# AlanLiangC/SPSNet

Hardware: NVIDIA B200
Metric: IA-SSD SA-backbone scenes/s (16k pts) (higher is better)
Workload: dtype fp16 operands / fp32 accumulate (split-fp16 hi+lo for K <= 64 chains and all Conv1d GEMMs); fp32 + int32 sampling

## Files before the change

spsnet_b200/csrc/sa_mma.cu:

```cuda
#include "sa_mma_common.cuh"
#include <stdlib.h>

namespace spsk {

template <int G, bool PROF, bool NP>
__global__ void __launch_bounds__(128 * G + 64 - (NP ? 32 : 0), G == 1 ? (NP ? 4 : 3) : 1)
sa_mma_kernel(const __grid_constant__ SaArgs a) {
    constexpr int W_PROD = NP ? -1 : 4 * G, W_MMA = NP ? 4 * G : 4 * G + 1;
    extern __shared__ __align__(128) uint8_t smem[];
    uint64_t *bars = reinterpret_cast<uint64_t *>(smem);
    uint32_t *tmem_slot = reinterpret_cast<uint32_t *>(smem + MM_HDR - 16);
    uint8_t *xa = smem + MM_HDR;
    uint8_t *xb = xa + a.xa_bytes;
    uint8_t *wst = xb + a.xb_bytes;
    const uint32_t bar0 = smem_u32(bars);
    auto W_FULL = [&](int s) { return bar0 + 8u * s; };
    auto W_EMPTY = [&](int s) { return bar0 + 8u * (MM_MAX_STAGES + s); };
    auto ACC_FULL = [&](int i) { return bar0 + 8u * (2 * MM_MAX_STAGES + i); };
    auto ACC_EMPTY = [&](int i) { return bar0 + 8u * (2 * MM_MAX_STAGES + 4 + i); };
    auto XR = [&](int buf, int c) { return bar0 + 8u * (2 * MM_MAX_STAGES + 8 + buf * MM_MAX_XC + c); };
    auto WL_FULL = [&](int s) { return bar0 + 8u * (2 * MM_MAX_STAGES + 8 + 2 * MM_MAX_XC + s); };
    auto WL_EMPTY = [&](int s) { return bar0 + 8u * (3 * MM_MAX_STAGES + 8 + 2 * MM_MAX_XC + s); };
    const uint32_t HID_DONE = bar0 + 8u * (4 * MM_MAX_STAGES + 8 + 2 * MM_MAX_XC);

// ... 39 lines not shown
                    { const long long t0 = pf.now(); mbar_wait(bar0 + ((R.z >> 10) & 1023u), ((R.z >> 20) ^ ((R.z >> 21) & tpar) ^ 1u) & 1u); pf.add(PF_PROD_W_EMPTY, t0); }
                    if (leader) {
                        const uint32_t full = bar0 + (R.z & 1023u), bytes = R.y & 0xFFFFu;
                        if (bytes == 0u || (PROF && (a.abl & 1) && tcount > 0u)) {
                            mbar_arrive(full);
                        } else {
                            mbar_expect_tx(full, bytes);
                            bulk_g2s(bar0 + ((R.y >> 16) << 4), a.wtiles + R.x, bytes, full);
                        }
                    }
                    __syncwarp();
                }
            }
            pf.flush(a.prof);
        } else {
            ProfT<PROF> pf;
            pf.init(a.prof != nullptr && leader);
            uint32_t tcount = 0;
            int ws = 0, ls = 0;
            uint32_t wph = 0u, lph = 0u;
            uint8_t *lst = ((nL - 2) & 1) ? xb : xa;
            for (int tile = blockIdx.x; tile < a.ntiles; tile += gridDim.x, ++tcount) {
                for (int l = 0; l < nL; ++l) {
                    const SaLayer &Ly = a.L[l];
                    const bool lring = a.lstages > 0 && l == nL - 1;
                    if (lring) { const long long t0 = pf.now(); mbar_wait(HID_DONE, tcount & 1u); pf.add(PF_PROD_HID, t0); }
                    for (int cci = 0; cci < Ly.n_cc; ++cci) {
                        const int cc = chunk_of(l, cci, Ly.n_cc);
                        const int ncols = min(128, Ly.cpad - cc * 128);
                        for (int kc = 0; kc < Ly.n_kc; ++kc) {
                            const int kw = min(64, Ly.wk - kc * 64);
                            const uint32_t bytes = (uint32_t)(ncols * kw * 2);
                            const uint8_t *src = a.wtiles + wtile_off(Ly, cc, kc, ncols);
                            uint32_t full, empty, dst, ph;
                            if (!lring) {
                                ph = wph;
                                full = W_FULL(ws); empty = W_EMPTY(ws); dst = smem_u32(wst + (size_t)ws * MM_STAGE_BYTES);
                                if (++ws == a.nstages) { ws = 0; wph ^= 1u; }
                            } else {
                                ph = lph;
                                full = WL_FULL(ls); empty = WL_EMPTY(ls); dst = smem_u32(lst + (size_t)ls * MM_STAGE_BYTES);
                                if (++ls == a.lstages) { ls = 0; lph ^= 1u; }
                            }
                            { const long long t0 = pf.now(); mbar_wait(empty, ph ^ 1u); pf.add(PF_PROD_W_EMPTY, t0); }
                            if (leader) {
                                mbar_expect_tx(full, bytes);
                                bulk_g2s(dst, src, bytes, full);
                            }
                            __syncwarp();
                        }
                    }
                }
            }
            pf.flush(a.prof);
        }
    } else if (warp == W_MMA) {
        if (a.narrow) {
            const bool leader = elect_one();
            if (NP && leader) {
                mbar_expect_tx(W_FULL(0), (uint32_t)a.w_total);
                for (int off = 0; off < a.w_total; off += MM_STAGE_BYTES) {
                    const int bytes = min(MM_STAGE_BYTES, a.w_total - off);
                    bulk_g2s(smem_u32(wst + off), a.wtiles + off, (uint32_t)bytes, W_FULL(0));
                }
            }
            uint32_t x_lo[MM_MAX_LAYERS], x_hi[MM_MAX_LAYERS], w_lo[MM_MAX_LAYERS], idesc[MM_MAX_LAYERS], tstride[MM_MAX_LAYERS];
            int nv[MM_MAX_LAYERS], nk1[MM_MAX_LAYERS], nk2[MM_MAX_LAYERS], nxc[MM_MAX_LAYERS], wkl[MM_MAX_LAYERS];
#pragma unroll
            for (int l = 0; l < MM_MAX_LAYERS; ++l) {
                const SaLayer &Ly = a.L[l < nL ? l : 0];
                const bool last = (l == nL - 1);
                x_lo[l] = umma_desc_lo(smem_u32((l & 1) ? xb : xa), 128u);
                x_hi[l] = umma_desc_hi((uint32_t)Ly.xw * 16u);
                w_lo[l] = umma_desc_lo(smem_u32(wst + Ly.w_off), 128u);
                tstride[l] = (uint32_t)(Ly.cpad * 64 * 2) >> 4;
                idesc[l] = last ? umma_idesc(128, MM_ROWS) : umma_idesc(128, Ly.cpad);
                nv[l] = Ly.vk >> 4;
                nk1[l] = a.split ? (Ly.kpad >> 4) : 0x7FFFFFFF;
                nk2[l] = a.split ? 2 * (Ly.kpad >> 4) : 0x7FFFFFFF;
                nxc[l] = Ly.n_xc;
                wkl[l] = Ly.wk;
            }
            mbar_wait(W_FULL(0), 0u);
            uint32_t job = 0;
            uint32_t xph[2] = {0u, 0u};
            const uint32_t nbmask = (uint32_t)a.nbuf - 1u;
            for (int tile = blockIdx.x; tile < a.ntiles; tile += gridDim.x) {
#pragma unroll
                for (int l = 0; l < MM_MAX_LAYERS; ++l) {
                    if (l < nL && l >= a.l0_fused) {
                        const bool last = (l == nL - 1);
                        const int buf = (int)(job & nbmask);
                        const uint32_t use = job >> a.nbuf_log2;
                        if (use > 0) mbar_wait(ACC_EMPTY(buf), (use - 1) & 1u);
                        for (int c = 0; c < nxc[l]; ++c) {
                            mbar_wait(XR(l & 1, c), (xph[l & 1] >> c) & 1u);
                            xph[l & 1] ^= (1u << c);
                        }
                        tc_fence_after();
                        if (leader) {
                            const uint32_t d_tmem = tmem_base + (uint32_t)(buf * 128);
                            for (int v = 0; v < nv[l]; ++v) {
                                const int xblk = v >= nk2[l] ? v - nk2[l] : v;
                                const int wblk = v >= nk1[l] ? v - nk1[l] : v;
                                const int kc = wblk >> 2, jj = wblk & 3;
                                const uint32_t kw = (uint32_t)min(64, wkl[l] - kc * 64);
                                const uint32_t wl = w_lo[l] + (uint32_t)kc * tstride[l] + 16u * (uint32_t)jj;
                                const uint32_t wh = umma_desc_hi(kw * 16u);
                                const uint32_t xl = x_lo[l] + 16u * (uint32_t)xblk;
                                if (!last) umma_f16_lohi(d_tmem, xl, x_hi[l], wl, wh, idesc[l], v ? 1u : 0u);
                                else umma_f16_lohi(d_tmem, wl, wh, xl, x_hi[l], idesc[l], v ? 1u : 0u);
                            }
                            umma_commit(ACC_FULL(buf));
                        }
                        __syncwarp();
                        ++job;
                    }
                }
            }
        } else if (a.sched_n > 0) {
            const bool leader = elect_one();
            ProfT<PROF> pf;
            pf.init(a.prof != nullptr && leader);
            const long long t_start = pf.now();
            uint32_t job = 0, tpar = 0u;
            const uint32_t nbmask = (uint32_t)a.nbuf - 1u;
            const int nent = a.sched_n;
            const uint32_t smem_base16 = bar0 >> 4;
            uint4 E = a.sched[0], R = a.ring[0];
            for (int tile = blockIdx.x; tile < a.ntiles; tile += gridDim.x, tpar ^= 1u) {
                int buf = 0;
                uint32_t d_tmem = tmem_base;
                for (int e = 0; e < nent; ++e) {
                    const int en = e + 1 < nent ? e + 1 : 0;
                    const uint4 En = a.sched[en], Rn = a.ring[en];
                    const uint32_t f = E.w;
                    if (f & SCH_FIRST_KC) {
                        buf = (int)(job & nbmask);
                        const uint32_t use = job >> a.nbuf_log2;
                        if (use > 0) { const long long t0 = pf.now(); mbar_wait(ACC_EMPTY(buf), (use - 1) & 1u); pf.add(PF_MMA_ACC_EMPTY, t0); }
                        d_tmem = tmem_base + (uint32_t)(buf * 128);
                    }
                    { const long long t0 = pf.now(); mbar_wait(bar0 + (R.z & 1023u), ((R.z >> 20) ^ ((R.z >> 21) & tpar)) & 1u); pf.add(PF_MMA_W_FULL, t0); }
                    if (R.z & (1u << 22)) {
                        const long long t0 = pf.now();
                        mbar_wait(bar0 + (R.w & 1023u), ((R.z >> 23) ^ ((R.z >> 24) & tpar)) & 1u);
                        if (R.z & (1u << 25)) mbar_wait(bar0 + (R.w >> 10), ((R.z >> 26) ^ ((R.z >> 27) & tpar)) & 1u);
                        pf.add(PF_MMA_XR, t0);
                    }
                    tc_fence_after();
                    if (leader) {
                        const long long t_i = pf.now();
                        const int nk16 = (PROF && (a.abl & 8) && (f & 15u)) ? 1 : (int)(f & 15u);
                        if (nk16) {
                            const uint32_t x_lo = E.x + smem_base16;
                            const uint32_t w_lo = (((smem_base16 + (R.y >> 16)) & 0x3FFFu) | ((128u >> 4) << 16));
                            const uint32_t w_lo2 = w_lo + ((f >> 16) & 2047u) - 64u;
                            const uint32_t x_hi = E.z & 0xFFFFu, w_hi = E.z >> 16;
                            const uint32_t acc0 = (f & SCH_FIRST_KC) ? 0u : 1u;
                            const int n1 = nk16 < 4 ? nk16 : 4;
                            if (!(f & SCH_LAST_LAYER)) {
                                umma_f16_lohi(d_tmem, x_lo, x_hi, w_lo, w_hi, E.y, acc0);
                                for (int j = 1; j < n1; ++j) umma_f16_lohi(d_tmem, x_lo + 16u * j, x_hi, w_lo + 16u * j, w_hi, E.y, 1u);
                                for (int j = 4; j < nk16; ++j) umma_f16_lohi(d_tmem, x_lo + 16u * j, x_hi, w_lo2 + 16u * j, w_hi, E.y, 1u);
                            } else {
                                umma_f16_lohi(d_tmem, w_lo, w_hi, x_lo, x_hi, E.y, acc0);
// ... 56 lines not shown
                            } else if (lring) {
                                { const long long t0 = pf.now(); mbar_wait(WL_FULL(ls), lph); pf.add(PF_MMA_W_FULL, t0); }
                                wbase = smem_u32(lst + (size_t)ls * MM_STAGE_BYTES);
                                wempty = WL_EMPTY(ls);
                                if (++ls == a.lstages) { ls = 0; lph ^= 1u; }
                            } else {
                                { const long long t0 = pf.now(); mbar_wait(W_FULL(ws), wph); pf.add(PF_MMA_W_FULL, t0); }
                                wbase = smem_u32(wst + (size_t)ws * MM_STAGE_BYTES);
                                wempty = W_EMPTY(ws);
                                if (++ws == a.nstages) { ws = 0; wph ^= 1u; }
                            }
                            const int nk16 = kw >> 4;
                            if (cci == 0) {
                                int need = (kc * 4 + nk16 - 1) >> 2;
                                if (a.split) need = Ly.n_xc - 1;
                                while (xwait <= need) {
                                    const long long t0 = pf.now();
                                    mbar_wait(XR(xbuf, xwait), (xph[xbuf] >> xwait) & 1u);
                                    pf.add(PF_MMA_XR, t0);
                                    xph[xbuf] ^= (1u << xwait);
                                    ++xwait;
                                }
                            }
                            tc_fence_after();
                            if (leader) {
                                const long long t_i = pf.now();
                                const uint32_t w_lo = umma_desc_lo(wbase, 128u);
                                const uint32_t w_hi = umma_desc_hi((uint32_t)kw * 16u);
                                const uint32_t x_lo = x_lo0 + (uint32_t)kc * 64u;
                                if (nk16 == 4 && !a.split) {
                                    if (!last) {
#pragma unroll
                                        for (int j = 0; j < 4; ++j)
                                            umma_f16_lohi(d_tmem, x_lo + 16u * j, x_hi, w_lo + 16u * j, w_hi, idesc, (kc | j) ? 1u : 0u);
                                    } else {
#pragma unroll
                                        for (int j = 0; j < 4; ++j)
                                            umma_f16_lohi(d_tmem, w_lo + 16u * j, w_hi, x_lo + 16u * j, x_hi, idesc, (kc | j) ? 1u : 0u);
                                    }
                                } else {
                                    for (int j = 0; j < nk16; ++j) {
                                        const int wb = kc * 4 + j;
                                        const uint32_t wl = w_lo + 16u * (uint32_t)j;
                                        auto issue = [&](int xblk, uint32_t acc) {
                                            const uint32_t xl = x_lo0 + 16u * (uint32_t)xblk;
                                            if (!last) umma_f16_lohi(d_tmem, xl, x_hi, wl, w_hi, idesc, acc);
                                            else umma_f16_lohi(d_tmem, wl, w_hi, xl, x_hi, idesc, acc);
                                        };
                                        if (!a.split) issue(wb, wb ? 1u : 0u);
                                        else if (wb < nk1) { issue(wb, wb ? 1u : 0u); issue(nk1 + wb, 1u); }
                                        else issue(wb - nk1, 1u);
                                    }
                                }
                                pf.add(PF_MMA_ISSUE, t_i);
                                const long long t_c = pf.now();
                                if (!a.resident) umma_commit(wempty);
                                if (kc == Ly.n_kc - 1) {
                                    umma_commit(ACC_FULL(buf));
                                    if (a.lstages > 0 && l == nL - 2 && cci == Ly.n_cc - 1) umma_commit(HID_DONE);
                                }
                                pf.add(PF_MMA_COMMIT, t_c);
                            }
                            __syncwarp();
                        }
                    }
                }
            }
            pf.add(PF_MMA_TOTAL, t_start);
            pf.flush(a.prof);
        }
    } else {
        ProfT<PROF> pf;
        pf.init(a.prof != nullptr && tid == 0);
        const long long t_start = pf.now();
        uint32_t job = 0;
        const uint32_t lane_field = (uint32_t)((warp & 3) * 32) << 16;
        const int r = tid & 127;
        const uint32_t grp = (uint32_t)(tid >> 7);
        const uint32_t row_off = (uint32_t)(r & 7) * 16u;
        const int first_tile = blockIdx.x;
        uint32_t prev_last_job = 0;
        bool have_prev = false;
        if (a.l0_fused) mbar_wait(W_FULL(0), 0u);
        int jn = 0;
        if (grp == 0 && first_tile < a.ntiles) {
            const long long grow = (long long)first_tile * MM_ROWS + r;
            if (grow < a.rows) jn = __ldg(a.idx + grow);
        }
        for (int tile = first_tile; tile < a.ntiles; tile += gridDim.x) {
            const long long t_g = pf.now();
            if (G == 2 && grp == 0 && have_prev) {
                const int pb = (int)(prev_last_job & ((uint32_t)a.nbuf - 1u));
                mbar_wait(ACC_FULL(pb), (prev_last_job >> a.nbuf_log2) & 1u);
            }
            if (grp == 0) {
                const SaLayer &L0 = a.L[0];
                const uint32_t sbo = (uint32_t)L0.xw * 16u;
                uint8_t *xrow = xa + (size_t)(r >> 3) * sbo + row_off;
                const long long grow = (long long)tile * MM_ROWS + r;
                const bool ok = grow < a.rows;
                const int j = jn;
                {
                    const long long gnext = grow + (long long)gridDim.x * MM_ROWS;
                    if (gnext < a.rows) jn = __ldg(a.idx + gnext);
                }
                long long q = 0;
                int bb = 0;
                if (ok) { q = grow >> a.ns_log2; bb = (int)(q / a.m); }
                float dx = 0.f, dy = 0.f, dz = 0.f;
                if (a.use_xyz && ok) {
                    const float *p = a.xyz + ((size_t)bb * a.n + j) * 3;
                    const float *ctr = a.new_xyz + (size_t)q * 3;
                    dx = __fsub_rn(__ldg(p), __ldg(ctr));
                    dy = __fsub_rn(__ldg(p + 1), __ldg(ctr + 1));
                    dz = __fsub_rn(__ldg(p + 2), __ldg(ctr + 2));
                }
                const uint4 zero = make_uint4(0, 0, 0, 0);
                if (!a.split) {
                    const int nch = L0.kpad >> 3;
                    const int fch = a.cpad8 >> 3;
                    const uint4 *trow = fch ? reinterpret_cast<const uint4 *>(a.twin + (ok ? ((size_t)bb * a.n + j) * a.ldtwin : 0)) : nullptr;
                    int c = 0;
                    if (fch > 8) {
                        const uint32_t xdst = smem_u32(xrow);
                        for (; c < fch; ++c) cp_async16(xdst + (uint32_t)c * 128u, trow + c, ok ? 16u : 0u);
                        cp_async_commit();
                    } else {
                        uint4 t[8];
#pragma unroll
                        for (int u = 0; u < 8; ++u) t[u] = (ok && u < fch) ? __ldg(trow + u) : zero;
#pragma unroll
                        for (int u = 0; u < 8; ++u)
                            if (u < fch) *reinterpret_cast<uint4 *>(xrow + (size_t)u * 128) = t[u];
                        c = fch;
                    }
                    if (a.use_xyz) {
                        *reinterpret_cast<uint4 *>(xrow + (size_t)c * 128) = make_uint4(pack_h2(dx, dy), pack_h2(dz, 0.f), 0u, 0u);
                        ++c;
                    }
                    for (; c < nch; ++c) *reinterpret_cast<uint4 *>(xrow + (size_t)c * 128) = zero;
                } else {
                    float y[16];
#pragma unroll
                    for (int i = 0; i < 16; ++i) y[i] = 0.f;
                    if (ok) {
#pragma unroll
                        for (int c = 0; c < 8; ++c)
                            if (c < a.c_feat) y[c] = __ldg(a.feat32 + ((size_t)bb * a.c_feat + c) * a.n + j);
                    }
                    if (a.c_feat) { y[8] = dx; y[9] = dy; y[10] = dz; }
                    else { y[0] = dx; y[1] = dy; y[2] = dz; }
                    if (a.l0_fused) {
                        const float *w0 = reinterpret_cast<const float *>(wst + a.l0_off);
                        const int c0n = L0.cpad;
                        float h[32];
#pragma unroll
                        for (int c = 0; c < 32; c += 4) {
                            const float4 bv = c < c0n ? *reinterpret_cast<const float4 *>(w0 + 16 * c0n + c) : make_float4(0.f, 0.f, 0.f, 0.f);
                            h[c] = bv.x; h[c + 1] = bv.y; h[c + 2] = bv.z; h[c + 3] = bv.w;
                        }
                        const int xo = a.c_feat ? 8 : 0;
#pragma unroll
                        for (int k = 0; k < 16; ++k) {
                            if (k < a.c_feat || (k >= xo && k < xo + 3)) {
                                const float yk = y[k];
#pragma unroll
                                for (int c = 0; c < 32; c += 4) {
                                    if (c < c0n) {
                                        const float4 wv = *reinterpret_cast<const float4 *>(w0 + k * c0n + c);
                                        h[c] = fmaf(yk, wv.x, h[c]); h[c + 1] = fmaf(yk, wv.y, h[c + 1]);
                                        h[c + 2] = fmaf(yk, wv.z, h[c + 2]); h[c + 3] = fmaf(yk, wv.w, h[c + 3]);
                                    }
                                }
                            }
                        }
                        const SaLayer &L1 = a.L[1];
                        uint8_t *x1 = xb + (size_t)(r >> 3) * ((uint32_t)L1.xw * 16u) + row_off;
                        uint8_t *x1lo = x1 + (size_t)(L1.kpad >> 3) * 128;
#pragma unroll
                        for (int g = 0; g < 4; ++g) {
                            if (8 * g < c0n) {
                                float t8[8];
#pragma unroll
                                for (int i = 0; i < 8; ++i) t8[i] = fmaxf(h[8 * g + i], 0.f);
                                uint4 hi, lo;
                                split8(t8, hi, lo);
                                *reinterpret_cast<uint4 *>(x1 + (size_t)g * 128) = hi;
                                *reinterpret_cast<uint4 *>(x1lo + (size_t)g * 128) = lo;
                            }
                        }
                        fence_proxy_async();
                        for (int c = 0; c < L1.n_xc; ++c) mbar_arrive(XR(1, c));
                    } else {
                    const int nch = L0.kpad >> 3;
                    uint8_t *xlo = xrow + (size_t)nch * 128;
                    uint4 hi, lo;
                    split8(y, hi, lo);
                    *reinterpret_cast<uint4 *>(xrow) = hi;
                    *reinterpret_cast<uint4 *>(xlo) = lo;
                    if (nch > 1) {
                        split8(y + 8, hi, lo);
                        *reinterpret_cast<uint4 *>(xrow + 128) = hi;
                        *reinterpret_cast<uint4 *>(xlo + 128) = lo;
                    }
                    }
                }
                if (!a.l0_fused) {
                    if (!a.split && (a.cpad8 >> 3) > 8) cp_async_wait<0>();
                    fence_proxy_async();
                    for (int c = 0; c < L0.n_xc; ++c) mbar_arrive(XR(0, c));
                }
            }
            pf.add(PF_EPI_GATHER, t_g);
            for (int l = a.l0_fused; l < nL - 1; ++l) {
                const SaLayer &Ly = a.L[l];
                const SaLayer &Ln = a.L[l + 1];
                const int obuf = (l + 1) & 1;
                uint8_t *xo = obuf ? xb : xa;
                const uint32_t sbo = (uint32_t)Ln.xw * 16u;
                uint8_t *xrow = xo + (size_t)(r >> 3) * sbo + row_off;
                const float *bias = a.bias + Ly.bias_off;
                for (int cc = 0; cc < Ly.n_cc; ++cc, ++job) {
                    if (G == 2 && (job & 1u) != grp) continue;
                    const int ncols = min(128, Ly.cpad - cc * 128);
                    const int buf = (int)(job & ((uint32_t)a.nbuf - 1u));
                    { const long long t0 = pf.now(); mbar_wait(ACC_FULL(buf), (job >> a.nbuf_log2) & 1u); pf.add(PF_EPI_WAIT_HID, t0); }
                    tc_fence_after();
                    const long long t_w = pf.now();
                    const uint32_t taddr = tmem_base + lane_field + (uint32_t)(buf * 128);
                    float hmx = 0.f;
                    if (!a.split) {
                        for (int h0 = 0; h0 < ncols; h0 += 64) {
                            const int hend = min(ncols, h0 + 64);
                            int c0 = (PROF && (a.abl & 2)) ? hend : h0;
                            for (; c0 + 32 <= hend; c0 += 32) {
                                float v[32];
                                tmem_ld32(taddr + (uint32_t)c0, v);
                                const int col = cc * 128 + c0;
                                store_hidden16(v, bias + col, xrow + (size_t)(col >> 3) * 128, hmx);
                                store_hidden16(v + 16, bias + col + 16, xrow + (size_t)((col >> 3) + 2) * 128, hmx);
                            }
                            if (c0 < hend) {
                                float v[16];
                                tmem_ld16(taddr + (uint32_t)c0, v);
                                const int col = cc * 128 + c0;
                                store_hidden16(v, bias + col, xrow + (size_t)(col >> 3) * 128, hmx);
                            }
                            fence_proxy_async();
                            mbar_arrive(XR(obuf, (cc * 128 + h0) >> 6));
                        }
                    } else {
                        uint8_t *xlo = xrow + (size_t)(Ln.kpad >> 3) * 128;
                        int c0 = 0;
                        for (; c0 + 32 <= ncols; c0 += 32) {
                            float v[32];
                            tmem_ld32(taddr + (uint32_t)c0, v);
                            store_hidden16_split(v, bias + c0, xrow + (size_t)(c0 >> 3) * 128, xlo + (size_t)(c0 >> 3) * 128, hmx);
                            store_hidden16_split(v + 16, bias + c0 + 16, xrow + (size_t)((c0 >> 3) + 2) * 128, xlo + (size_t)((c0 >> 3) + 2) * 128, hmx);
                        }
                        if (c0 < ncols) {
                            float v[16];
                            tmem_ld16(taddr + (uint32_t)c0, v);
                            store_hidden16_split(v, bias + c0, xrow + (size_t)(c0 >> 3) * 128, xlo + (size_t)(c0 >> 3) * 128, hmx);
                        }
                        fence_proxy_async();
                        for (int c = 0; c < Ln.n_xc; ++c) mbar_arrive(XR(obuf, c));
                    }
                    if (hmx > FP16_MAX && a.ovf) atomicOr(a.ovf, a.ovf_bit);
                    tc_fence_before();
                    mbar_arrive(ACC_EMPTY(buf));
                    pf.add(PF_EPI_WORK_HID, t_w);
                }
            }
            if (a.stats) {
                const SaLayer &Ly = a.L[nL - 1];
                const long long left = a.rows - (long long)tile * MM_ROWS;
                const int nv = left < MM_ROWS ? (int)left : MM_ROWS;
                double *slice = a.stats + (size_t)(blockIdx.x * G + (G == 2 ? grp : 0u)) * (size_t)Ly.cpad * 2;
                for (int cci = 0; cci < Ly.n_cc; ++cci, ++job) {
                    if (G == 2 && (job & 1u) != grp) continue;
                    const int cc = chunk_of(nL - 1, cci, Ly.n_cc);
                    const int buf = (int)(job & ((uint32_t)a.nbuf - 1u));
                    mbar_wait(ACC_FULL(buf), (job >> a.nbuf_log2) & 1u);
                    tc_fence_after();
                    stats_chunk(tmem_base + lane_field + (uint32_t)(buf * 128), nv, slice + (size_t)(cc * 128 + r) * 2);
                    tc_fence_before();
                    mbar_arrive(ACC_EMPTY(buf));
                }
            } else
            {
                const SaLayer &Ly = a.L[nL - 1];
                const float *bias = a.bias + Ly.bias_off;
                const long long q0 = ((long long)tile * MM_ROWS) >> a.ns_log2;
                const long long qmax = (long long)a.b * a.m;
                const int ns = a.nsample;
                const long long bb0 = q0 / a.m;
                const int p0 = (int)(q0 - bb0 * a.m);
                const size_t sstride = (size_t)a.c_total * a.m;
                for (int cci = 0; cci < Ly.n_cc; ++cci, ++job) {
                    if (G == 2 && (job & 1u) != grp) continue;
                    const int cc = chunk_of(nL - 1, cci, Ly.n_cc);
                    const int buf = (int)(job & ((uint32_t)a.nbuf - 1u));
                    { const long long t0 = pf.now(); mbar_wait(ACC_FULL(buf), (job >> a.nbuf_log2) & 1u); pf.add(PF_EPI_WAIT_POOL, t0); }
                    tc_fence_after();
                    const long long t_w = pf.now();
                    const int ch = cc * 128 + r;
                    const bool w32 = a.out != nullptr && ch < a.cout_last;
                    const bool w16 = a.out16 != nullptr && ch < a.n16;
                    const float bv = __ldg(bias + ch);
                    PoolOut o;
                    o.bv = bv; o.w32 = w32; o.w16 = w16;
                    o.outc = a.out + ((size_t)bb0 * a.c_total + a.co_off + (w32 ? ch : 0)) * a.m + (size_t)p0;
                    o.out16 = a.out16 + (size_t)q0 * a.ld16 + a.co16 + (w16 ? ch : 0);
                    o.ld16 = a.ld16; o.o16lo = a.o16lo; o.q = q0; o.qmax = qmax; o.m = a.m; o.p = p0; o.scene_stride = sstride;
                    const uint32_t taddr = tmem_base + lane_field + (uint32_t)(buf * 128);
                    if (ns == 32) pool_chunk<32>(taddr, o);
                    else if (ns == 16) pool_chunk<16>(taddr, o);
                    else pool_chunk_any(taddr, o, ns);
                    if (o.mx16 > FP16_MAX && a.ovf) atomicOr(a.ovf, a.ovf_bit);
                    tc_fence_before();
                    mbar_arrive(ACC_EMPTY(buf));
                    pf.add(PF_EPI_WORK_POOL, t_w);
                }
            }
            prev_last_job = job - 1u;
            have_prev = true;
        }
        pf.add(PF_EPI_TOTAL, t_start);
        pf.flush(a.prof);
    }

    tc_fence_before();
    __syncthreads();
    if (warp == W_MMA) {
        tc_fence_after();
        tmem_dealloc(tmem_base, (uint32_t)a.tmem_cols);
    }
}

__global__ void __launch_bounds__(256)
make_twin_kernel(int c, int n, int cpad8, const float *__restrict__ in, __half *__restrict__ out, unsigned int *ovf) {
    __shared__ float tile[32][33];
    const int b = blockIdx.z;
    const int n0 = blockIdx.x * 32, c0 = blockIdx.y * 32;
    const int tx = threadIdx.x & 31, ty = threadIdx.x >> 5;
    for (int i = ty; i < 32; i += 8) {
        const int ci = c0 + i, ni = n0 + tx;
        tile[i][tx] = (ci < c && ni < n) ? __ldg(in + ((size_t)b * c + ci) * n + ni) : 0.f;
    }
    __syncthreads();
    for (int i = ty; i < 32; i += 8) {
        const int ni = n0 + i, ci = c0 + tx;
        if (ni < n && ci < cpad8) {
            out[((size_t)b * n + ni) * cpad8 + ci] = __float2half_rn(tile[tx][i]);
            if (fabsf(tile[tx][i]) > FP16_MAX && ovf) atomicOr(ovf, 1u);
        }
    }
}

static unsigned long long *g_sa_prof = nullptr;

struct SaTuning {
    int max_stages, max_ctas, grid_mult;
    int abl;
    bool no_lring, no_sched, rot, no_narrow, one_group, no_double;
    SaTuning() {
        auto geti = [](const char *name, int dflt) { const char *e = getenv(name); return e ? atoi(e) : dflt; };
        max_stages = max(2, min(MM_MAX_STAGES, geti("SPSK_SA_MAX_STAGES", MM_MAX_STAGES)));
        max_ctas = max(1, min(4, geti("SPSK_SA_MAX_CTAS", 4)));
        grid_mult = max(1, min(8, geti("SPSK_SA_GRID_MULT", 1)));
        abl = geti("SPSK_SA_ABL", 0);
        no_lring = getenv("SPSK_SA_NO_LRING") != nullptr;
        no_sched = getenv("SPSK_SA_NO_SCHED") != nullptr;
        rot = getenv("SPSK_SA_ROT") != nullptr;
        no_narrow = getenv("SPSK_SA_NO_NARROW") != nullptr;
        no_double = getenv("SPSK_SA_NO_DOUBLE") != nullptr;
        one_group = getenv("SPSK_SA_ONE_GROUP") != nullptr;
    }
};
static const SaTuning &sa_tuning() {
    static const SaTuning t;
    return t;
}

struct SaPlan {
    SaLayer L[MM_MAX_LAYERS];
    int xa_bytes, xb_bytes, w_total, l0_off, resident, nstages, lstages, ctas, tmem_cols, nbuf, smem, sched_n;
};

constexpr int PR_HDR_BYTES = 2048;

static int sa_plan(const spsk_sa_mma_desc *d, SaPlan *P) {
    const int nL = d->nlayers;
    const bool pair = d->pair != 0;
    SPSK_REQUIRE(nL >= 1 && nL <= MM_MAX_LAYERS, SPSK_ERR_UNSUPPORTED, "sa_mma: nlayers=%d (1..%d)", nL, MM_MAX_LAYERS);
    const int split = d->split ? 1 : 0;
    int w_off = 0, b_off = 0;
    P->xa_bytes = P->xb_bytes = 0;
    for (int l = 0; l < nL; ++l) {
        const bool last = l == nL - 1;
        const int kpad = d->kpad[l], cpad = d->cpad[l];
        SPSK_REQUIRE(kpad >= 16 && kpad % 16 == 0 && kpad <= 1024, SPSK_ERR_UNSUPPORTED, "sa_mma: layer %d kpad=%d", l, kpad);
        SPSK_REQUIRE(cpad >= 16 && cpad % (last ? 128 : 16) == 0 && cpad <= (last ? 4096 : 1024), SPSK_ERR_UNSUPPORTED,
                     "sa_mma: layer %d cpad=%d", l, cpad);
        SPSK_REQUIRE(last || cpad == d->kpad[l + 1], SPSK_ERR_INVALID_ARG, "sa_mma: layer %d cpad != next kpad", l);
        SPSK_REQUIRE(!split || (kpad <= 64 && (last || cpad <= 64)), SPSK_ERR_UNSUPPORTED, "sa_mma: split arithmetic needs every width <= 64");
        SPSK_REQUIRE(!pair || (!split && (!last || cpad % 256 == 0)), SPSK_ERR_UNSUPPORTED, "sa_mma: pair kernel needs plain arithmetic and a last cpad multiple of 256");
        SaLayer &Ly = P->L[l];
        Ly.kpad = kpad; Ly.cpad = cpad;
        Ly.n_cc = pair ? (cpad + 255) / 256 : (cpad + 127) / 128;
        Ly.xw = split ? 2 * kpad : kpad;
        Ly.vk = split ? 3 * kpad : kpad;
        Ly.wk = split ? 2 * kpad : kpad;
        Ly.n_kc = (Ly.wk + 63) / 64;
        Ly.n_xc = (Ly.xw + 63) / 64;
        Ly.w_off = w_off; Ly.bias_off = b_off;
        w_off += Ly.wk * cpad * 2;
        b_off += cpad;
        const int xbytes = Ly.xw * MM_ROWS * 2;
        if (l & 1) P->xb_bytes = max(P->xb_bytes, xbytes); else P->xa_bytes = max(P->xa_bytes, xbytes);
    }
    P->w_total = w_off;
    P->l0_off = 0;
    if (d->l0_fused) {
        SPSK_REQUIRE(split && nL >= 2 && d->cpad[0] <= 32 && !pair, SPSK_ERR_UNSUPPORTED, "sa_mma: layer-0 fusion needs a split chain of >= 2 layers with cpad[0] <= 32");
        P->l0_off = w_off;
        P->w_total = w_off + (16 * d->cpad[0] + d->cpad[0]) * 4;
        P->w_total = (P->w_total + 15) & ~15;
    }
    const int xtot = (pair ? PR_HDR_BYTES : MM_HDR) + P->xa_bytes + P->xb_bytes;
    const int sm_bytes = 228 * 1024;
    auto fits = [&](int ctas, int *resident, int *nstages, int *smem) {
        const int per = (sm_bytes / ctas - 1024) & ~127;
        if (xtot + P->w_total <= per) { *resident = 1; *nstages = 1; *smem = xtot + P->w_total; return true; }
        const int st = (per - xtot) / MM_STAGE_BYTES;
        if (st < 2) return false;
        const int cap = sa_tuning().max_stages;
        *resident = 0; *nstages = st > cap ? cap : st; *smem = xtot + *nstages * MM_STAGE_BYTES;
        return true;
    };
    int ctas = 0;
    const int cmax = pair ? 1 : sa_tuning().max_ctas;
    bool one_job_per_layer = true;
    for (int l = 0; l < nL; ++l) one_job_per_layer = one_job_per_layer && P->L[l].n_cc == 1;
    for (int c = cmax; c >= 1; --c) {
        int res, st, sm;
        if (!fits(c, &res, &st, &sm)) continue;
        if (c == 4 && !(res && one_job_per_layer && !d->l0_fused)) continue;
        ctas = c; P->resident = res; P->nstages = st; P->smem = sm;
        break;
    }
    SPSK_REQUIRE(ctas >= 1, SPSK_ERR_UNSUPPORTED, "sa_mma: activation tiles do not fit shared memory (layer widths too large)");
    P->ctas = ctas;
    P->lstages = 0;
    if (pair && P->resident) {
        P->resident = 0;
        P->nstages = min(MM_MAX_STAGES, max(2, (P->smem - xtot) / MM_STAGE_BYTES));
        P->smem = xtot + P->nstages * MM_STAGE_BYTES;
    }
    if (!P->resident && P->nstages < 4 && nL >= 2 && !sa_tuning().no_lring) {
// ... 176 lines not shown
    using namespace spsk;
    SPSK_REQUIRE(d && nparts, SPSK_ERR_INVALID_ARG, "sa_mma: null descriptor");
    SPSK_REQUIRE(!d->pair, SPSK_ERR_UNSUPPORTED, "sa_mma: the batch-statistics pass runs on the single-CTA kernel (pair == 0)");
    SaPlan P;
    if (int rc = sa_plan(d, &P)) return rc;
    const long long rows = (long long)d->b * d->m * d->nsample;
    const long long ntiles = (rows + MM_ROWS - 1) / MM_ROWS;
    const long long slots = (long long)SPSK_NUM_SMS * P.ctas * sa_tuning().grid_mult;
    const long long grid = ntiles < slots ? ntiles : slots;
    const bool two_groups = P.ctas == 1 && !sa_tuning().one_group;
    *nparts = (int)(grid * (two_groups ? 2 : 1));
    return SPSK_OK;
}

extern "C" int spsk_sa_mma_forward(const spsk_sa_mma_desc *d, spsk_stream_t stream) {
    using namespace spsk;
    SPSK_REQUIRE(d, SPSK_ERR_INVALID_ARG, "sa_mma: null descriptor");
    SPSK_REQUIRE(d->wtiles && d->bias && (d->out_cm || d->out16 || d->stats), SPSK_ERR_INVALID_ARG, "sa_mma: null weights / no output");
    SPSK_REQUIRE(!d->stats || !d->pair, SPSK_ERR_UNSUPPORTED, "sa_mma: the batch-statistics pass runs on the single-CTA kernel (pair == 0)");
    SPSK_REQUIRE(d->nsample >= 1 && d->nsample <= MM_ROWS && (d->nsample & (d->nsample - 1)) == 0, SPSK_ERR_UNSUPPORTED,
                 "sa_mma: nsample=%d must be a power of two <= %d", d->nsample, MM_ROWS);
    SPSK_REQUIRE(d->b >= 0 && d->n >= 1 && d->m >= 0 && d->c_feat >= 0, SPSK_ERR_INVALID_ARG, "sa_mma: bad sizes");
    SPSK_REQUIRE(d->idx && d->xyz && d->new_xyz, SPSK_ERR_INVALID_ARG, "sa_mma: null gather source");
    SaPlan P;
    if (int rc = sa_plan(d, &P)) return rc;
    SaArgs a{};
    a.nlayers = d->nlayers;
    for (int l = 0; l < d->nlayers; ++l) a.L[l] = P.L[l];
    a.b = d->b; a.n = d->n; a.m = d->m; a.nsample = d->nsample;
    a.ns_log2 = 0;
    while ((1 << a.ns_log2) < d->nsample) ++a.ns_log2;
    a.c_feat = d->c_feat;
    a.use_xyz = d->use_xyz ? 1 : 0;
    a.split = d->split ? 1 : 0;
    if (a.split) {
        SPSK_REQUIRE(d->c_feat <= 8 && (d->c_feat == 0 || d->features), SPSK_ERR_UNSUPPORTED, "sa_mma: split arithmetic takes <= 8 fp32 feature channels");
        SPSK_REQUIRE(d->kpad[0] == 16, SPSK_ERR_INVALID_ARG, "sa_mma: split kpad[0]=%d must be 16 ([f0..f7 | x y z 0..])", d->kpad[0]);
        a.feat32 = d->features;
        a.cpad8 = d->c_feat ? 8 : 0;
    } else {
        a.cpad8 = (d->c_feat + 7) / 8 * 8;
        SPSK_REQUIRE(d->c_feat == 0 || (d->twin && d->ldtwin >= a.cpad8 && d->ldtwin % 8 == 0 && (reinterpret_cast<uintptr_t>(d->twin) & 15) == 0),
                     SPSK_ERR_INVALID_ARG, "sa_mma: twin must be a 16-byte aligned (b, n, ldtwin) fp16 tensor with ldtwin %% 8 == 0 and >= c_feat");
        SPSK_REQUIRE(d->kpad[0] >= a.cpad8 + (a.use_xyz ? 8 : 0), SPSK_ERR_INVALID_ARG, "sa_mma: kpad[0]=%d too small for %d feature + xyz channels",
                     d->kpad[0], a.cpad8);
        a.twin = reinterpret_cast<const __half *>(d->twin);
        a.ldtwin = d->ldtwin;
    }
    a.rows = (long long)d->b * d->m * d->nsample;
    if (a.rows == 0) return SPSK_OK;
    const long long ntiles = (a.rows + MM_ROWS - 1) / MM_ROWS;
    SPSK_REQUIRE(ntiles <= 0x7FFFFFFF, SPSK_ERR_UNSUPPORTED, "sa_mma: too many rows");
    a.ntiles = (int)ntiles;
    a.lstages = P.lstages;
    a.sched_n = P.sched_n;
    a.rot_last = (P.L[d->nlayers - 1].n_cc > 1 && sa_tuning().rot) ? 1 : 0;
    a.l0_fused = d->l0_fused ? 1 : 0;
    a.l0_off = P.l0_off;
    SPSK_REQUIRE(!a.l0_fused || P.resident, SPSK_ERR_UNSUPPORTED, "sa_mma: layer-0 fusion needs the chain resident in shared memory");
    a.narrow = P.resident && !sa_tuning().no_narrow;
    for (int l = 0; l < d->nlayers; ++l)
        if (P.L[l].n_cc != 1) a.narrow = 0;
    a.nstages = P.nstages; a.resident = P.resident; a.w_total = P.w_total; a.tmem_cols = P.tmem_cols; a.nbuf = P.nbuf;
    a.nbuf_log2 = P.nbuf == 4 ? 2 : (P.nbuf == 2 ? 1 : 0);
    a.xa_bytes = P.xa_bytes; a.xb_bytes = P.xb_bytes;
    a.xyz = d->xyz; a.new_xyz = d->new_xyz; a.idx = d->idx;
    a.wtiles = reinterpret_cast<const uint8_t *>(d->wtiles); a.bias = d->bias;
    SPSK_REQUIRE((reinterpret_cast<uintptr_t>(d->wtiles) & 15) == 0, SPSK_ERR_INVALID_ARG, "sa_mma: wtiles must be 16-byte aligned");
    a.cout_last = d->cout_last;
    SPSK_REQUIRE(d->cout_last >= 1 && d->cout_last <= d->cpad[d->nlayers - 1], SPSK_ERR_INVALID_ARG, "sa_mma: cout_last outside the last layer");
    a.out = d->out_cm; a.c_total = d->c_total; a.co_off = d->co_off;
    if (a.out) SPSK_REQUIRE(d->co_off >= 0 && d->co_off + d->cout_last <= d->c_total, SPSK_ERR_INVALID_ARG, "sa_mma: channel window outside c_total");
    a.out16 = reinterpret_cast<__half *>(d->out16); a.ld16 = d->ld16; a.co16 = d->co16; a.n16 = d->n16; a.o16lo = d->o16lo;
    if (a.out16 && d->o16lo)
        SPSK_REQUIRE(d->o16lo > 0 && d->o16lo + d->co16 + d->n16 <= d->ld16, SPSK_ERR_INVALID_ARG, "sa_mma: residual columns outside ld16");
    if (a.out16)
        SPSK_REQUIRE(d->n16 >= d->cout_last && d->n16 <= d->cpad[d->nlayers - 1] && d->co16 >= 0 && d->co16 + d->n16 <= d->ld16, SPSK_ERR_INVALID_ARG,
                     "sa_mma: fp16 output window [co16, co16 + n16) outside ld16 or wider than the last layer");
    a.prof = g_sa_prof;
    a.ovf = fp16_overflow_word();
    a.ovf_bit = 1u << (d->ovf_tag & 31);
    a.stats = d->stats;
    a.abl = sa_tuning().abl;
    if (d->pair) {
        a.ntiles = (int)((a.rows + 255) / 256);
        return spsk_sa_mma_pair_launch(a, P.smem, as_stream(stream));
    }
    const int mult = sa_tuning().grid_mult;
    const int slots = SPSK_NUM_SMS * P.ctas * mult;
    const int grid = a.ntiles < slots ? a.ntiles : slots;
    if (a.sched_n > 0) {
        a.sched_n = build_schedule(a, !sa_tuning().no_double);
        if (a.sched_n > 0) a.rot_last = 0;
    }
    const bool two_groups = P.ctas == 1 && !sa_tuning().one_group;
    if (a.stats) {
        SPSK_REQUIRE((reinterpret_cast<uintptr_t>(d->stats) & 15) == 0, SPSK_ERR_INVALID_ARG, "sa_mma: stats must be 16-byte aligned");
        SPSK_REQUIRE(d->stats_parts >= grid * (two_groups ? 2 : 1), SPSK_ERR_INVALID_ARG, "sa_mma: stats holds %d parts, this launch writes %d",
                     d->stats_parts, grid * (two_groups ? 2 : 1));
        a.out = nullptr; a.out16 = nullptr;
        const size_t bytes = (size_t)grid * (two_groups ? 2 : 1) * (size_t)P.L[d->nlayers - 1].cpad * 2 * sizeof(double);
        cudaError_t e = cudaMemsetAsync(d->stats, 0, bytes, as_stream(stream));
        if (e != cudaSuccess) return cuda_fail(e, "sa_mma: cudaMemsetAsync(stats)");
    }
#define SPSK_SA_LAUNCH(GV, PV)                                                                                               \
    do {                                                                                                                    \
        static SmemAttrOnce attr;                                                                                           \
        if (int rc = attr.ensure(reinterpret_cast<const void *>(sa_mma_kernel<GV, PV, false>), 227 * 1024, "sa_mma_kernel")) return rc; \
        sa_mma_kernel<GV, PV, false><<<grid, 128 * GV + 64, P.smem, as_stream(stream)>>>(a);                                    \
    } while (0)
    if (P.ctas == 4) {
        SPSK_REQUIRE(a.narrow && a.resident, SPSK_ERR_UNSUPPORTED, "sa_mma: the 4-CTA shape needs the resident narrow issue loop (unset SPSK_SA_NO_NARROW)");
        static SmemAttrOnce attr4, attr4p;
        if (a.prof) {
            if (int rc = attr4p.ensure(reinterpret_cast<const void *>(sa_mma_kernel<1, true, true>), 227 * 1024, "sa_mma_kernel<np,prof>")) return rc;
            sa_mma_kernel<1, true, true><<<grid, 160, P.smem, as_stream(stream)>>>(a);
        } else {
            if (int rc = attr4.ensure(reinterpret_cast<const void *>(sa_mma_kernel<1, false, true>), 227 * 1024, "sa_mma_kernel<np>")) return rc;
            sa_mma_kernel<1, false, true><<<grid, 160, P.smem, as_stream(stream)>>>(a);
        }
    } else if (two_groups) {
        if (a.prof) SPSK_SA_LAUNCH(2, true); else SPSK_SA_LAUNCH(2, false);
    } else {
        if (a.prof) SPSK_SA_LAUNCH(1, true); else SPSK_SA_LAUNCH(1, false);
    }
#undef SPSK_SA_LAUNCH
    SPSK_LAUNCH_CHECK("sa_mma_kernel");
    return SPSK_OK;
}
```

spsnet_b200/csrc/sa_mma_common.cuh:

```cuda
#pragma once
#include "mma_ptx.cuh"

namespace spsk {

constexpr int MM_ROWS = 128;
constexpr int MM_THREADS = 192;
constexpr int MM_STAGE_BYTES = 16384;
constexpr int MM_MAX_LAYERS = 4;
constexpr int MM_MAX_STAGES = 8;
constexpr int MM_HDR = 1024;
constexpr int MM_SCHED_MAX = 104;
constexpr uint32_t SCH_FIRST_KC = 1u << 4;
constexpr uint32_t SCH_LAST_KC = 1u << 5;
constexpr uint32_t SCH_LRING_FIRST = 1u << 11;
constexpr uint32_t SCH_HID_DONE = 1u << 12;
constexpr uint32_t SCH_LAST_LAYER = 1u << 13;
constexpr int MM_MAX_XC = 16;

struct SaLayer {
    int kpad;
    int cpad;
    int n_cc;
    int xw;
    int vk;
    int wk;
    int n_kc;
    int n_xc;
    int w_off;
    int bias_off;
};

struct SaArgs {
    int nlayers;
    SaLayer L[MM_MAX_LAYERS];
    int b, n, m, nsample, ns_log2;
    int c_feat, cpad8, ldtwin, use_xyz, split;
    long long rows;
    int ntiles;
    int nstages, resident, w_total, tmem_cols, nbuf, nbuf_log2;
    int l0_fused, l0_off;
    int rot_last;
    int sched_n;
    int narrow;
    int lstages;
    int xa_bytes, xb_bytes;
    const float *xyz, *new_xyz, *feat32;
    const __half *twin;
    const int *idx;
    const uint8_t *wtiles;
    const float *bias;
    float *out;
    int c_total, co_off, cout_last;
    __half *out16;
    int ld16, co16, n16, o16lo;
    unsigned long long *prof;
    unsigned int *ovf;
    unsigned int ovf_bit;
    int abl;
    double *stats;
    uint4 sched[MM_SCHED_MAX];
    uint4 ring[MM_SCHED_MAX];
};

__device__ __forceinline__ int wtile_off(const SaLayer &Ly, int cc, int kc, int ncols) {
    return Ly.w_off + (128 * cc * Ly.wk + ncols * 64 * kc) * 2;
}

__device__ __forceinline__ void store_hidden16(const float *v, const float *bias16, uint8_t *dst, float &mx) {
    const float4 *b4 = reinterpret_cast<const float4 *>(bias16);
    uint32_t h[8];
#pragma unroll
    for (int i = 0; i < 4; ++i) {
        const float4 bb = __ldg(b4 + i);
        const float s0 = v[4 * i] + bb.x, s1 = v[4 * i + 1] + bb.y, s2 = v[4 * i + 2] + bb.z, s3 = v[4 * i + 3] + bb.w;
        mx = fmaxf(fmaxf(mx, s0), s1);
        mx = fmaxf(fmaxf(mx, s2), s3);
        h[2 * i] = pack_h2_relu(s0, s1);
        h[2 * i + 1] = pack_h2_relu(s2, s3);
    }
    *reinterpret_cast<uint4 *>(dst) = make_uint4(h[0], h[1], h[2], h[3]);
    *reinterpret_cast<uint4 *>(dst + 128) = make_uint4(h[4], h[5], h[6], h[7]);
}
__device__ __forceinline__ void split8(const float *y, uint4 &hi, uint4 &lo) {
    uint32_t h[4], l[4];
#pragma unroll
    for (int i = 0; i < 4; ++i) {
        const __half2 hh = __floats2half2_rn(y[2 * i], y[2 * i + 1]);
        const float2 hf = __half22float2(hh);
        h[i] = *reinterpret_cast<const uint32_t *>(&hh);
        l[i] = pack_h2(y[2 * i] - hf.x, y[2 * i + 1] - hf.y);
    }
    hi = make_uint4(h[0], h[1], h[2], h[3]);
    lo = make_uint4(l[0], l[1], l[2], l[3]);
}
__device__ __forceinline__ void store_hidden16_split(const float *v, const float *bias16, uint8_t *dst_hi, uint8_t *dst_lo, float &mx) {
    const float4 *b4 = reinterpret_cast<const float4 *>(bias16);
    float y[16];
#pragma unroll
    for (int i = 0; i < 4; ++i) {
        const float4 bb = __ldg(b4 + i);
        y[4 * i] = fmaxf(v[4 * i] + bb.x, 0.f); y[4 * i + 1] = fmaxf(v[4 * i + 1] + bb.y, 0.f);
        y[4 * i + 2] = fmaxf(v[4 * i + 2] + bb.z, 0.f); y[4 * i + 3] = fmaxf(v[4 * i + 3] + bb.w, 0.f);
        mx = fmaxf(fmaxf(mx, y[4 * i]), y[4 * i + 1]);
        mx = fmaxf(fmaxf(mx, y[4 * i + 2]), y[4 * i + 3]);
    }
    uint4 h0, l0, h1, l1;
    split8(y, h0, l0);
    split8(y + 8, h1, l1);
    *reinterpret_cast<uint4 *>(dst_hi) = h0;
    *reinterpret_cast<uint4 *>(dst_hi + 128) = h1;
    *reinterpret_cast<uint4 *>(dst_lo) = l0;
    *reinterpret_cast<uint4 *>(dst_lo + 128) = l1;
}

struct PoolOut {
    float mx16 = 0.f;
    float bv;
    bool w32, w16;
    float *outc;
    __half *out16;
    int ld16, o16lo;
    long long q, qmax;
    int m, p;
    size_t scene_stride;
    __device__ __forceinline__ void emit(float run) {
        const float y = fmaxf(run + bv, 0.f);
        if (q < qmax) {
            if (w32) *outc = y;
            if (w16) {
                mx16 = fmaxf(mx16, y);
                const __half h = __float2half_rn(y);
                *out16 = h;
                if (o16lo > 0) out16[o16lo] = __float2half_rn(y - __half2float(h));
            }
        }
        ++q;
        ++outc;
        out16 += ld16;
        if (++p == m) { p = 0; outc += scene_stride - (size_t)m; }
    }
};
template <int NS, int NCOLS = MM_ROWS>
__device__ __forceinline__ void pool_chunk(uint32_t taddr, PoolOut &o) {
    float run = -3.0e38f;
#pragma unroll 1
    for (int c0 = 0; c0 < NCOLS; c0 += 32) {
        float v[32];
        tmem_ld32(taddr + (uint32_t)c0, v);
#pragma unroll
        for (int i = 0; i < 32; ++i) {
            run = fmaxf(run, v[i]);
            if (((i + 1) % NS) == 0) { o.emit(run); run = -3.0e38f; }
        }
    }
}
static __device__ __noinline__ void pool_chunk_any(uint32_t taddr, PoolOut &o, int ns, int ncols = MM_ROWS) {
    float run = -3.0e38f;
#pragma unroll 1
    for (int c0 = 0; c0 < ncols; c0 += 16) {
        float v[16];
        tmem_ld16(taddr + (uint32_t)c0, v);
#pragma unroll
        for (int i = 0; i < 16; ++i) {
            run = fmaxf(run, v[i]);
            if (((c0 + i + 1) & (ns - 1)) == 0) { o.emit(run); run = -3.0e38f; }
        }
    }
}

static_assert(sizeof(SaArgs) <= 4096, "SaArgs travels in the kernel parameters: keep it within the classic 4 KB limit");

static __device__ __forceinline__ void stats_chunk(uint32_t taddr, int nv, double *cell) {
    float s = 0.f, q = 0.f;
#pragma unroll 1
    for (int c0 = 0; c0 < nv; c0 += 32) {
        float v[32];
        tmem_ld32(taddr + (uint32_t)c0, v);
#pragma unroll
        for (int i = 0; i < 32; ++i) {
            const float x = (c0 + i < nv) ? v[i] : 0.f;
            s += x;
            q = fmaf(x, x, q);
        }
    }
    double2 acc = *reinterpret_cast<double2 *>(cell);
    acc.x += (double)s;
    acc.y += (double)q;
    *reinterpret_cast<double2 *>(cell) = acc;
}

enum { PF_MMA_TOTAL = 0, PF_MMA_ACC_EMPTY, PF_MMA_W_FULL, PF_MMA_XR, PF_PROD_W_EMPTY, PF_PROD_HID, PF_EPI_TOTAL, PF_EPI_GATHER,
       PF_EPI_WAIT_HID, PF_EPI_WORK_HID, PF_EPI_WAIT_POOL, PF_EPI_WORK_POOL, PF_MMA_ISSUE, PF_MMA_COMMIT, PF_COUNT };
template <bool ON>
struct ProfT {
    unsigned long long acc[PF_COUNT];
    bool on;
    __device__ __forceinline__ void init(bool enable) {
        on = enable;
#pragma unroll
        for (int i = 0; i < PF_COUNT; ++i) acc[i] = 0ull;
    }
    __device__ __forceinline__ long long now() const { return on ? clock64() : 0ll; }
    __device__ __forceinline__ void add(int k, long long t0) { if (on) acc[k] += (unsigned long long)(clock64() - t0); }
    __device__ __forceinline__ void flush(unsigned long long *dst) const {
        if (!on) return;
        for (int i = 0; i < PF_COUNT; ++i)
            if (acc[i]) atomicAdd(dst + i, acc[i]);
    }
};
template <>
struct ProfT<false> {
    __device__ __forceinline__ void init(bool) {}
    __device__ __forceinline__ long long now() const { return 0ll; }
    __device__ __forceinline__ void add(int, long long) {}
    __device__ __forceinline__ void flush(unsigned long long *) const {}
};
using Prof = ProfT<true>;


}
```

Before: 11950.

## Replicate narrow last-layer weights so all TMEM lanes pool disjoint row spans

```diff
diff --git a/spsnet_b200/csrc/sa_mma.cu b/spsnet_b200/csrc/sa_mma.cu
--- a/spsnet_b200/csrc/sa_mma.cu
+++ b/spsnet_b200/csrc/sa_mma.cu
@@ -145,6 +145,20 @@
                 wkl[l] = Ly.wk;
             }
             mbar_wait(W_FULL(0), 0u);
+            if (a.rep_log2 > 0) {
+                const SaLayer &Ly = a.L[nL - 1];
+                const int span = MM_ROWS >> a.rep_log2;
+                for (int kc = 0; kc < Ly.n_kc; ++kc) {
+                    uint4 *t = reinterpret_cast<uint4 *>(wst + wtile_off(Ly, 0, kc, MM_ROWS));
+                    const int n16 = (span * min(64, Ly.wk - kc * 64) * 2) >> 4;
+                    for (int i = tid & 31; i < n16; i += 32) {
+                        const uint4 v = t[i];
+                        for (int rr = 1; rr < (1 << a.rep_log2); ++rr) t[rr * n16 + i] = v;
+                    }
+                }
+                fence_proxy_async();
+                __syncwarp();
+            }
             uint32_t job = 0;
             uint32_t xph[2] = {0u, 0u};
             const uint32_t nbmask = (uint32_t)a.nbuf - 1u;
@@ -367,8 +381,9 @@
         uint32_t prev_last_job = 0;
         bool have_prev = false;
         if (a.l0_fused) mbar_wait(W_FULL(0), 0u);
+        const bool gload = !(PROF && (a.abl & 32));
         int jn = 0;
-        if (grp == 0 && first_tile < a.ntiles) {
+        if (gload && grp == 0 && first_tile < a.ntiles) {
             const long long grow = (long long)first_tile * MM_ROWS + r;
             if (grow < a.rows) jn = __ldg(a.idx + grow);
         }
@@ -384,16 +399,17 @@
                 uint8_t *xrow = xa + (size_t)(r >> 3) * sbo + row_off;
                 const long long grow = (long long)tile * MM_ROWS + r;
                 const bool ok = grow < a.rows;
+                const bool okl = ok && gload;
                 const int j = jn;
                 {
                     const long long gnext = grow + (long long)gridDim.x * MM_ROWS;
-                    if (gnext < a.rows) jn = __ldg(a.idx + gnext);
+                    if (gload && gnext < a.rows) jn = __ldg(a.idx + gnext);
                 }
                 long long q = 0;
                 int bb = 0;
                 if (ok) { q = grow >> a.ns_log2; bb = (int)(q / a.m); }
                 float dx = 0.f, dy = 0.f, dz = 0.f;
-                if (a.use_xyz && ok) {
+                if (a.use_xyz && okl) {
                     const float *p = a.xyz + ((size_t)bb * a.n + j) * 3;
                     const float *ctr = a.new_xyz + (size_t)q * 3;
                     dx = __fsub_rn(__ldg(p), __ldg(ctr));
@@ -408,12 +424,12 @@
                     int c = 0;
                     if (fch > 8) {
                         const uint32_t xdst = smem_u32(xrow);
-                        for (; c < fch; ++c) cp_async16(xdst + (uint32_t)c * 128u, trow + c, ok ? 16u : 0u);
+                        for (; c < fch; ++c) cp_async16(xdst + (uint32_t)c * 128u, trow + c, okl ? 16u : 0u);
                         cp_async_commit();
                     } else {
                         uint4 t[8];
 #pragma unroll
-                        for (int u = 0; u < 8; ++u) t[u] = (ok && u < fch) ? __ldg(trow + u) : zero;
+                        for (int u = 0; u < 8; ++u) t[u] = (okl && u < fch) ? __ldg(trow + u) : zero;
 #pragma unroll
                         for (int u = 0; u < 8; ++u)
                             if (u < fch) *reinterpret_cast<uint4 *>(xrow + (size_t)u * 128) = t[u];
@@ -428,7 +444,7 @@
                     float y[16];
 #pragma unroll
                     for (int i = 0; i < 16; ++i) y[i] = 0.f;
-                    if (ok) {
+                    if (okl) {
 #pragma unroll
                         for (int c = 0; c < 8; ++c)
                             if (c < a.c_feat) y[c] = __ldg(a.feat32 + ((size_t)bb * a.c_feat + c) * a.n + j);
@@ -576,7 +592,10 @@
             {
                 const SaLayer &Ly = a.L[nL - 1];
                 const float *bias = a.bias + Ly.bias_off;
-                const long long q0 = ((long long)tile * MM_ROWS) >> a.ns_log2;
+                const int span = MM_ROWS >> a.rep_log2;
+                const int rep_i = r >> (7 - a.rep_log2);
+                const int rr = r - rep_i * span;
+                const long long q0 = ((long long)tile * MM_ROWS + rep_i * span) >> a.ns_log2;
                 const long long qmax = (long long)a.b * a.m;
                 const int ns = a.nsample;
                 const long long bb0 = q0 / a.m;
@@ -589,7 +608,7 @@
                     { const long long t0 = pf.now(); mbar_wait(ACC_FULL(buf), (job >> a.nbuf_log2) & 1u); pf.add(PF_EPI_WAIT_POOL, t0); }
                     tc_fence_after();
                     const long long t_w = pf.now();
-                    const int ch = cc * 128 + r;
+                    const int ch = cc * 128 + rr;
                     const bool w32 = a.out != nullptr && ch < a.cout_last;
                     const bool w16 = a.out16 != nullptr && ch < a.n16;
                     const float bv = __ldg(bias + ch);
@@ -598,10 +617,12 @@
                     o.outc = a.out + ((size_t)bb0 * a.c_total + a.co_off + (w32 ? ch : 0)) * a.m + (size_t)p0;
                     o.out16 = a.out16 + (size_t)q0 * a.ld16 + a.co16 + (w16 ? ch : 0);
                     o.ld16 = a.ld16; o.o16lo = a.o16lo; o.q = q0; o.qmax = qmax; o.m = a.m; o.p = p0; o.scene_stride = sstride;
-                    const uint32_t taddr = tmem_base + lane_field + (uint32_t)(buf * 128);
-                    if (ns == 32) pool_chunk<32>(taddr, o);
-                    else if (ns == 16) pool_chunk<16>(taddr, o);
-                    else pool_chunk_any(taddr, o, ns);
+                    const uint32_t taddr = tmem_base + lane_field + (uint32_t)(buf * 128 + rep_i * span);
+                    if (!(PROF && (a.abl & 16))) {
+                        if (ns == 32) pool_chunk<32>(taddr, o, span);
+                        else if (ns == 16) pool_chunk<16>(taddr, o, span);
+                        else pool_chunk_any(taddr, o, ns, span);
+                    }
                     if (o.mx16 > FP16_MAX && a.ovf) atomicOr(a.ovf, a.ovf_bit);
                     tc_fence_before();
                     mbar_arrive(ACC_EMPTY(buf));
@@ -648,7 +669,7 @@
 struct SaTuning {
     int max_stages, max_ctas, grid_mult;
     int abl;
-    bool no_lring, no_sched, rot, no_narrow, one_group, no_double;
+    bool no_lring, no_sched, rot, no_narrow, one_group, no_double, no_rep;
     SaTuning() {
         auto geti = [](const char *name, int dflt) { const char *e = getenv(name); return e ? atoi(e) : dflt; };
         max_stages = max(2, min(MM_MAX_STAGES, geti("SPSK_SA_MAX_STAGES", MM_MAX_STAGES)));
@@ -661,6 +682,7 @@
         no_narrow = getenv("SPSK_SA_NO_NARROW") != nullptr;
         no_double = getenv("SPSK_SA_NO_DOUBLE") != nullptr;
         one_group = getenv("SPSK_SA_ONE_GROUP") != nullptr;
+        no_rep = getenv("SPSK_SA_NO_REP") != nullptr;
     }
 };
 static const SaTuning &sa_tuning() {
@@ -1003,6 +1025,12 @@
     a.ovf_bit = 1u << (d->ovf_tag & 31);
     a.stats = d->stats;
     a.abl = sa_tuning().abl;
+    a.rep_log2 = 0;
+    if (a.narrow && !a.stats && !d->pair && !sa_tuning().no_rep) {
+        const int wch = max(a.cout_last, a.out16 ? a.n16 : 0);
+        const int span = max(wch <= 32 ? 32 : (wch <= 64 ? 64 : MM_ROWS), a.nsample);
+        a.rep_log2 = span == 32 ? 2 : (span == 64 ? 1 : 0);
+    }
     if (d->pair) {
         a.ntiles = (int)((a.rows + 255) / 256);
         return spsk_sa_mma_pair_launch(a, P.smem, as_stream(stream));
diff --git a/spsnet_b200/csrc/sa_mma_common.cuh b/spsnet_b200/csrc/sa_mma_common.cuh
--- a/spsnet_b200/csrc/sa_mma_common.cuh
+++ b/spsnet_b200/csrc/sa_mma_common.cuh
@@ -57,6 +57,7 @@
     unsigned int *ovf;
     unsigned int ovf_bit;
     int abl;
+    int rep_log2;
     double *stats;
     uint4 sched[MM_SCHED_MAX];
     uint4 ring[MM_SCHED_MAX];
@@ -141,10 +142,10 @@
     }
 };
 template <int NS, int NCOLS = MM_ROWS>
-__device__ __forceinline__ void pool_chunk(uint32_t taddr, PoolOut &o) {
+__device__ __forceinline__ void pool_chunk(uint32_t taddr, PoolOut &o, int ncols = NCOLS) {
     float run = -3.0e38f;
 #pragma unroll 1
-    for (int c0 = 0; c0 < NCOLS; c0 += 32) {
+    for (int c0 = 0; c0 < ncols; c0 += 32) {
         float v[32];
         tmem_ld32(taddr + (uint32_t)c0, v);
 #pragma unroll
```

New measurement: 12120 (median of 6 runs). +1.5%, better.
